# rust-bio/rust-bio

Measured on AMD Instinct MI355X. Metric: GCUPS (SW) + FM-index queries/sec, higher is better.
Workload: dtype int16; 1 GPU; 1000000 x 150 bp synthetic read pairs per GPU, Aligner::local affine-gap (-5,-1,+1,-1), score+coords+traceback ops (BASELINE configs[1]); pairs_per_gpu=1000000, read_len=150, parallelism=shard1

## Files before the change

### rust-bio_amd/csrc/sw_fill_pk16.inc

```
#include <type_traits>

#include "sw_kernels.h"

namespace bgsw {
namespace pk16 {

typedef uint32_t pk;

typedef short s16x2 __attribute__((ext_vector_type(2)));
typedef unsigned short u16x2 __attribute__((ext_vector_type(2)));
typedef _Float16 h16x2 __attribute__((ext_vector_type(2)));
__device__ __forceinline__ s16x2 as_s(pk v) { return __builtin_bit_cast(s16x2, v); }
__device__ __forceinline__ u16x2 as_u(pk v) { return __builtin_bit_cast(u16x2, v); }
__device__ __forceinline__ pk bits(s16x2 v) { return __builtin_bit_cast(pk, v); }
__device__ __forceinline__ pk bits(u16x2 v) { return __builtin_bit_cast(pk, v); }
__device__ __forceinline__ pk pk_adds(pk a, pk b) { return bits(__builtin_elementwise_add_sat(as_s(a), as_s(b))); }
__device__ __forceinline__ pk pk_max(pk a, pk b) { return bits(__builtin_elementwise_max(as_s(a), as_s(b))); }
__device__ __forceinline__ pk pk_max3h(pk a, pk b, pk c) {
    const h16x2 x = __builtin_bit_cast(h16x2, a), y = __builtin_bit_cast(h16x2, b), z = __builtin_bit_cast(h16x2, c);
    return __builtin_bit_cast(pk, __builtin_elementwise_maximum(__builtin_elementwise_maximum(x, y), z));
}
__device__ __forceinline__ pk pk_min(pk a, pk b) { return bits(__builtin_elementwise_min(as_s(a), as_s(b))); }
__device__ __forceinline__ pk pk_add_u16(pk a, pk b) { return bits((u16x2)(as_u(a) + as_u(b))); }
__device__ __forceinline__ pk pk_sub_u16(pk a, pk b) { return bits((u16x2)(as_u(a) - as_u(b))); }
__device__ __forceinline__ pk pk_subs_u16(pk a, pk b) { return bits(__builtin_elementwise_sub_sat(as_u(a), as_u(b))); }
__device__ __forceinline__ pk pk_mad_u16(pk a, pk b, pk c) { return bits((u16x2)(as_u(a) * as_u(b) + as_u(c))); }
__device__ __forceinline__ pk dup16(int32_t v) { return ((uint32_t)v & 0xffffu) | ((uint32_t)v << 16); }
__device__ __forceinline__ pk bfi(pk mask, pk a, pk b) { return (a & mask) | (b & ~mask); }
__device__ __forceinline__ pk nz_mask(pk v, pk one) { return pk_sub_u16(pk_subs_u16(one, v), one); }

template <int LP>
__device__ __forceinline__ void scan_first_max(int ll, int64_t& v, uint32_t& idx) {
#pragma unroll
    for (int off = 1; off < LP; off <<= 1) {
        const int64_t ov = __shfl_up(v, off, LP);
        const uint32_t oi = (uint32_t)__shfl_up((int)idx, off, LP);
        if (ll >= off && !(v > ov)) {
            v = ov;
            idx = oi;
        }
    }
}

constexpr int32_t kFloor16 = -2048;

enum { CZ = 0, CF = 1, CI = 2 };
template <int R, int LP, int MODE, int XP, int XS, int YP, int YS, bool LF = false, int FR = 0>
__device__ __forceinline__ void sw_fill_pk16_body(const SwArgs& a) {
    constexpr bool FAST = MODE == 0;
    constexpr int PW = 64 / LP;
    constexpr int NW = tb_words(R);
    constexpr int NH = (R + 2) / 3;
    constexpr bool NARROW = true, LOCAL = XP == CZ && XS == CZ && YP == CZ && YS == CZ;
    constexpr bool ROW0_ZERO = YP == CZ && YS == CZ;
    constexpr int SH = 4;
    constexpr int32_t NEGS = kFloor16 * 16;
    constexpr pk CLEAN = 0xfff0fff0u, FLOORK = 0x80008000u, ONE = 0x00010001u;
    static_assert(LP == 16 || LP == 32, "lanes per pair");
    static_assert(R >= 1 && R <= 12, "rows per lane");
    static_assert(!LF || LOCAL, "LF is a flavour of the local kernel");
    static_assert(FR >= 0 && FR <= 2 && (!FR || LF), "the frame is a cell of the LF flavour");
    (void)NARROW;
    (void)LOCAL;
    constexpr int kTileStride = 20;
    constexpr int kParkDw = 64 * (4 * R + NH + 1), kTileDw = 2 * 64 * kTileStride;
    constexpr int kWaveDw = kParkDw > kTileDw ? kParkDw : kTileDw;
    __shared__ __align__(16) pk s_lds[4 * kWaveDw];
    pk* const wave_lds = s_lds + (threadIdx.x >> 6) * kWaveDw;

    const int lane = threadIdx.x & 63;
    const uint32_t wv = blockIdx.x * (blockDim.x >> 6) + (threadIdx.x >> 6);
    if ((uint64_t)wv * 2 * PW >= a.n_pairs) return;
    if (MODE == 2 && a.len_stats && a.len_stats[0] == a.len_stats[2] && a.len_stats[1] == a.len_stats[3]) return;
    const int g = lane / LP, ll = lane % LP;
    const SwScoring sc = a.sc;
    const SwGeom geo = a.g;
    auto scl = [](int32_t v) -> int32_t { return max(v, kFloor16) * 16; };
    const int32_t go_s = sc.go * 16, xs_s = sc.xs <= kFloor16 ? -(1 << 30) : sc.xs * 16;
    (void)xs_s;
    constexpr int32_t K_XS = C_XS << 1, K_MATCH = C_MATCH << 1, K_SUBST = C_SUBST << 1, K_INS = C_INS << 1,
                      K_DEL = C_DEL << 1, K_XP = C_XP << 1;
    constexpr pk NOFLAG = 0xfffefffeu;
    const pk GE = dup16(sc.ge * 16);
    const pk GOT_I = dup16(sc.go * 16 + K_INS + 1), GOT_D = dup16(sc.go * 16 + K_DEL + 1);
    const pk MISK = dup16((sc.mismatch * 16) | K_SUBST);
    const pk DELTA = dup16(((sc.match * 16) | K_MATCH) - ((sc.mismatch * 16) | K_SUBST));
    const pk XS16 = dup16(scl(sc.xs)), YS16 = dup16(scl(sc.ys));
    const pk XSCAP = sc.xs <= kFloor16 ? FLOORK : 0x7fff7fffu, YSCAP = sc.ys <= kFloor16 ? FLOORK : 0x7fff7fffu;
    (void)XS16; (void)YS16; (void)XSCAP; (void)YSCAP;
    const pk MISC = dup16(-((sc.mismatch * 16) | K_SUBST));
    (void)MISC;
    auto fr = [](int32_t c) -> pk { return (uint32_t)c * 0x10001u; };
    const int32_t gF = -16 * sc.ge, BF = pk16_frame_bias(sc);
    const pk GF = fr(gF);
    const pk KGOI = fr(sc.go * 16 + K_INS + 1 + gF), KGOD = fr(sc.go * 16 + K_DEL + 1 + gF);
    const pk KSUB = fr(((sc.mismatch * 16) | K_SUBST) + 2 * gF);
    const pk KREB = fr(gF * (R - 1));
    (void)GF; (void)KGOI; (void)KGOD; (void)KSUB; (void)KREB;
    pk C16 = dup16(16), C32 = dup16(32), C1024 = dup16(1024);
    asm volatile("" : "+s"(C16), "+s"(C32), "+s"(C1024));

    const uint32_t pA = (2 * wv) * PW + g, pB = (2 * wv + 1) * PW + g;
    const bool okA = pA < a.n_pairs, okB = pB < a.n_pairs;
    uint32_t mA = 0, nA = 0, mB = 0, nB = 0;
    uint64_t xoA = 0, yoA = 0, xoB = 0, yoB = 0;
    const uint32_t* perm = a.slot_perm();
    if (okA) {
        const uint64_t r = a.pair0 + (perm ? perm[pA] : pA);
        xoA = a.x_off[r];
        yoA = a.y_off[r];
        mA = (uint32_t)(a.x_off[r + 1] - xoA);
        nA = (uint32_t)(a.y_off[r + 1] - yoA);
        if (len_over(geo, mA, nA)) mA = nA = 0;
    }
    if (okB) {
        const uint64_t r = a.pair0 + (perm ? perm[pB] : pB);
        xoB = a.x_off[r];
        yoB = a.y_off[r];
        mB = (uint32_t)(a.x_off[r + 1] - xoB);
        nB = (uint32_t)(a.y_off[r + 1] - yoB);
        if (len_over(geo, mB, nB)) mB = nB = 0;
    }
    const bool same = okA && okB && mA == mB && nA == nB;
    const bool two = okA && okB && !same;
    const bool m_last0 = LF || __all(!okA || mA % R == 0);
    if (MODE == 0 && !m_last0) return;
    if (MODE == 1 && m_last0) return;
    if (MODE == 2 && !__any(two)) return;
    const uint64_t job_words = tb_job_words(geo.nstrips, geo.nsteps, NW);

    auto do_pass = [&](const int pass) {
        const bool pair_ok = pass == 0 ? okA : two;
        const uint32_t P0 = pass == 0 ? pA : pB, P1 = (pass == 0 && !same) ? pA : pB;
        const uint32_t m = !pair_ok ? 0 : (pass == 0 ? mA : mB), n = !pair_ok ? 0 : (pass == 0 ? nA : nB);
        const uint64_t xs0 = pass == 0 ? xoA : xoB, ys0 = pass == 0 ? yoA : yoB;
        const uint64_t xs1 = (pass == 0 && !same) ? xoA : xoB, ys1 = (pass == 0 && !same) ? yoA : yoB;
        const uint8_t* x0 = a.x + xs0;
        const uint8_t* x1 = a.x + xs1;
        const bool packed = a.packed != 0;
        auto y_pair = [&](uint32_t col) -> pk {
            if (packed) return sym2(a.y, ys0 + col) | (sym2(a.y, ys1 + col) << 16);
            return (uint32_t)a.y[ys0 + col] | ((uint32_t)a.y[ys1 + col] << 16);
        };
        const uint32_t Q0 = pair_ok ? P0 : 0, Q1 = pair_ok ? P1 : 0;
        uint32_t* tb0 = (uint32_t*)a.tb + (size_t)(Q0 / PW) * job_words + ((Q0 % PW) * LP + ll) * 16u;
        uint32_t* tb1 = (uint32_t*)a.tb + (size_t)(Q1 / PW) * job_words + ((Q1 % PW) * LP + ll) * 16u;
        int32_t* aux0 = a.aux + (size_t)Q0 * geo.aux_stride;
        int32_t* aux1 = a.aux + (size_t)Q1 * geo.aux_stride;
        int32_t* gLx0 = aux0 + geo.off_Lx();
        int32_t* gLx1 = aux1 + geo.off_Lx();

        uint32_t m_w = m, n_w = n;
#pragma unroll
        for (int o = 32; o; o >>= 1) {
            m_w = max(m_w, (uint32_t)__shfl_xor((int)m_w, o));
            n_w = max(n_w, (uint32_t)__shfl_xor((int)n_w, o));
        }
        (void)m_w;
        n_w = (uint32_t)__builtin_amdgcn_readfirstlane((int)n_w);
        const uint32_t nsteps_w = n_w ? n_w + LP - 1 : 0;

        int32_t fold0;
        uint32_t lx0;
        col0_fold(sc, m, fold0, lx0);
        int32_t Sn0 = sc.ys;
        uint32_t Ly0 = n;
        int32_t S0n = 0;
        uint32_t sb0n = (ROW0_ZERO && n) ? row0_cell(sc, n).sbits : (uint32_t)TB_START;
        if (pair_ok && ll == 0) {
            const int32_t v = m ? (int32_t)col0_cell(sc, m, m, fold0).sbits : (int32_t)TB_START;
            aux0[0] = v;
            aux1[0] = v;
            if (m == 0) {
                if (LP == 16) {
                    *(uint8_t*)gLx0 = (uint8_t)lx0;
                    *(uint8_t*)gLx1 = (uint8_t)lx0;
                } else {
                    *(uint16_t*)gLx0 = (uint16_t)lx0;
                    *(uint16_t*)gLx1 = (uint16_t)lx0;
                }
            }
        }

        const uint32_t rb = (uint32_t)ll * R;
        const int32_t mrow = (int32_t)m - (int32_t)rb - 1;
        pk Sl[R], Dl[R], Il[R], SnR[R], SnB[R], Ly[R], px[R];
        uint64_t nib0S = 0, nib0I = 0;
        uint64_t xw0 = 0, xw1 = 0;
        if (packed && pair_ok && rb < m) {
            const uint32_t* p0 = (const uint32_t*)a.x + ((xs0 + rb) >> 4);
            const uint32_t* p1 = (const uint32_t*)a.x + ((xs1 + rb) >> 4);
            xw0 = (((uint64_t)p0[1] << 32) | p0[0]) >> (2 * ((uint32_t)(xs0 + rb) & 15u));
            xw1 = (((uint64_t)p1[1] << 32) | p1[0]) >> (2 * ((uint32_t)(xs1 + rb) & 15u));
        }
#pragma unroll
        for (int r = 0; r < R; r++) {
            const uint32_t i = rb + r + 1;
            px[r] = 0;
            Sl[r] = Dl[r] = Il[r] = SnR[r] = SnB[r] = FLOORK;
            Ly[r] = 0;
            if (pair_ok && i <= m) {
                px[r] = packed ? (((uint32_t)(xw0 >> (2 * r)) & 3u) | (((uint32_t)(xw1 >> (2 * r)) & 3u) << 16))
                               : ((uint32_t)x0[i - 1] | ((uint32_t)x1[i - 1] << 16));
                const Col0 c = col0_cell(sc, i, m, fold0);
                Sl[r] = dup16(scl(c.S));
                Il[r] = dup16(scl(c.I) | K_INS);
                nib0S |= (uint64_t)c.sbits << (4 * r);
                nib0I |= (uint64_t)c.ibits << (4 * r);
                if (YS != CI && c.S + sc.ys > NEG) {
                    SnR[r] = dup16(scl(c.S + sc.ys));
                    Ly[r] = dup16((int32_t)n);
                }
            }
        }
        pk diag0 = dup16((pair_ok && rb < m) ? scl(col0_S(sc, rb, m, fold0)) : NEGS);
        if (FR) {
            const int32_t off0 = BF + gF * ((int32_t)ll - 1);
#pragma unroll
            for (int r = 0; r < R; r++) {
                const pk o = fr(off0 + gF * r);
                Sl[r] = (pair_ok && rb + r + 1 <= m) ? Sl[r] + o : o;
                Il[r] += o;
                Dl[r] = 0;
            }
            diag0 = fr(off0 - gF) + ((pair_ok && rb < m) ? dup16(scl(col0_S(sc, rb, m, fold0))) : 0u);
        }

        pk S_out = FLOORK, I_out = FLOORK, cm_out = FLOORK, ca_out = 0, q_out = 0;
        pk ychunk = 0, ychunk_nx = 0;
        pk hwlast[NH];
#pragma unroll
        for (int k = 0; k < NH; k++) hwlast[k] = 0;
        pk lx_n = dup16((int32_t)lx0);
        pk* tileA = wave_lds + (0 * 64 + lane) * kTileStride;
        pk* tileB = wave_lds + (1 * 64 + lane) * kTileStride;
        uint32_t lxaccA = lx0 << (LP == 16 ? 24 : 16), lxaccB = lxaccA;
        if (pair_ok && (uint32_t)ll < n) ychunk_nx = y_pair((uint32_t)ll);

        auto merge_rows = [&](uint32_t blockbase) {
            const pk lybase = dup16((int32_t)(n - blockbase - 16u + (uint32_t)ll));
#pragma unroll
            for (int r = 0; r < R; r++) {
                const pk nr = pk_max(SnR[r], SnB[r] & CLEAN);
                const pk msk = nz_mask(nr ^ SnR[r], ONE);
                Ly[r] = bfi(msk, pk_add_u16(lybase, SnB[r] & 0x000f000fu), Ly[r]);
                SnR[r] = nr;
                SnB[r] = FLOORK;
            }
        };

        constexpr uint32_t tsteps = tb_tile_steps(NW);
        auto store_tile = [&](uint32_t s_any) {
            if (!pair_ok) return;
            const uint32_t off = (s_any / tsteps) * 1024u;
#pragma unroll
            for (int k = 0; k < 4; k++) {
                *(uint4*)&tb0[off + 4 * k] = *(const uint4*)&tileA[4 * k];
                *(uint4*)&tb1[off + 4 * k] = *(const uint4*)&tileB[4 * k];
            }
        };
        uint32_t s_all = pair_ok ? n + (uint32_t)ll : 0u;
#pragma unroll
        for (int o = 32; o; o >>= 1) s_all = min(s_all, (uint32_t)__shfl_xor((int)s_all, o));
        s_all = (uint32_t)__builtin_amdgcn_readfirstlane((int)s_all);
        auto run_steps = [&](auto mr_tag) {
        constexpr int MRk = decltype(mr_tag)::value;
        auto step = [&](auto allon_tag, auto fast_tag, const uint32_t s) {
            constexpr bool ALLON = decltype(allon_tag)::value;
            constexpr bool FB = decltype(fast_tag)::value;
            constexpr bool FOLD = XS != CI && !FB;
            if ((s & (LP - 1)) == 0) {
                ychunk = ychunk_nx;
                const uint32_t nb = s + LP + ll;
                if (pair_ok && nb < n) ychunk_nx = y_pair(nb);
            }
            pk S_up = (pk)wave_shr1((int)S_out, (int)S_out), I_up = (pk)wave_shr1((int)I_out, (int)I_out);
            if (FR) {
                S_up -= KREB;
                I_up -= KREB;
            }
            pk cm = FLOORK, ca = 0;
            if (FOLD) {
                cm = (pk)wave_shr1((int)cm_out, (int)cm_out);
                ca = (pk)wave_shr1((int)ca_out, (int)ca_out);
            }
            pk q = (pk)wave_shr1((int)q_out, (int)q_out);
            const uint32_t j = s + 1 - (uint32_t)ll;
            const bool col_ok = ALLON || (pair_ok && (j - 1) < n);
            const pk F0 = fr(BF + gF * (int32_t)s);
            (void)F0;
            if (ll == 0) {
                q = ychunk;
                S_up = FR ? F0 - GF : 0u;
                I_up = FR ? 0u : FLOORK;
                cm = FLOORK;
                ca = 0;
                if (!ROW0_ZERO && col_ok) {
                    const Row0 c = row0_cell(sc, j);
                    int32_t S0 = c.S;
                    uint32_t sb = c.sbits;
                    if (j == n && Sn0 > S0) {
                        S0 = Sn0;
                        sb = TB_YCLIP_SUFFIX;
                    } else if (S0 + sc.ys > Sn0) {
                        Sn0 = S0 + sc.ys;
                        Ly0 = n - j;
                    }
                    S0n = S0;
                    sb0n = sb;
                    S_up = dup16(scl(S0));
                }
            }
            ychunk = (pk)wave_shl1((int)ychunk, (int)ychunk);

            if (col_ok) {
                const pk sprio = dup16((int32_t)(15u - (s & 15u)));
                pk diag = diag0;
                diag0 = S_up;
                pk hw[NH];
                const pk ca_in = ca;
                pk cmk = cm | 0x000f000fu;
                pk snap = cmk;
                pk XKEY = dup16(K_XP);
                if (XP == CF || (XP == CZ && YP != CZ))
                    XKEY = dup16(scl(sc.xp + max(sc.yp, sc.go + sc.ge * ((int32_t)j - 1))) | K_XP);
#pragma unroll
                    for (int r = 0; r < R; r++) {
                        const bool maybe_m = MRk < 0 || r == MRk;
                        const bool is_m = MRk < 0 ? (r == mrow) : (r == MRk && mrow == MRk);
                        const pk e = pk_subs_u16(ONE, px[r] ^ q);
                        const pk Fr = F0 + (uint32_t)r * GF;
                        (void)Fr;
                        const pk m_key = FR == 2 ? pk_mad_u16(e, DELTA, diag) + KSUB
                                         : FR    ? pk_max(pk_mad_u16(e, DELTA, diag) + KSUB, Fr)
                                         : LF    ? pk_subs_u16(pk_mad_u16(e, DELTA, diag), MISC)
                                                 : pk_adds(diag, pk_mad_u16(e, DELTA, MISK));
                        const pk Iv_t = FR ? pk_max(I_up, S_up + KGOI) : pk_max(pk_adds(I_up, GE), pk_adds(S_up, GOT_I));
                        const pk Dv_t = FR ? pk_max(Dl[r], Sl[r] + KGOD) : pk_max(pk_adds(Dl[r], GE), pk_adds(Sl[r], GOT_D));
                        const pk Iv = Iv_t & NOFLAG, Dv = Dv_t & NOFLAG;
                        pk kb = FR == 2 ? pk_max3h(m_key, Fr, Dv_t) : pk_max(m_key, Dv_t);
                        if (XP != CI && !LF) kb = pk_max(kb, XKEY);
                        kb = FR == 2 ? pk_max3h(kb, Iv_t, Iv_t) : pk_max(kb, Iv_t);
                        if (FOLD && maybe_m)
                            kb = pk_max(kb, is_m ? ((cmk & CLEAN) | (0x00010001u * K_XS)) : FLOORK);
                        const pk best = kb & CLEAN;
                        diag = Sl[r];
                        Sl[r] = best;
                        Dl[r] = Dv;
                        Il[r] = Iv;
                        S_up = best;
                        I_up = Iv;
                        if (FOLD) {
                            if (maybe_m) snap = is_m ? cmk : snap;
                            const pk fv = XS == CZ ? best : pk_min(pk_adds(best, XS16), XSCAP);
                            cmk = pk_max(cmk, fv | (0x00010001u * (uint32_t)(14 - r)));
                        }
                        if (YS != CI) {
                            const pk t1 = YS == CZ ? best : pk_min(pk_adds(best, YS16), YSCAP);
                            SnB[r] = pk_max(SnB[r], FR ? best - (Fr - sprio) : t1 | sprio);
                        }
                        const pk c5 = pk_mad_u16(Dv_t & ONE, C16, (kb & 0x000e000eu) | (Iv_t & ONE));
                        if (r % 3 == 0)
                            hw[r / 3] = c5;
                        else
                            hw[r / 3] = pk_mad_u16(c5, r % 3 == 1 ? C32 : C1024, hw[r / 3]);
                    }
                if (FOLD) {
                    const pk mbase = dup16(mrow - 14);
                    const pk lo = cmk & 0x000f000fu, slo = snap & 0x000f000fu;
                    if (mrow >= 0 && mrow < R) {
                        const pk is15 = nz_mask(slo ^ 0x000f000fu, ONE);
                        lx_n = bfi(is15, pk_add_u16(slo, mbase), ca_in);
                        if (LP == 16) {
                            lxaccA = __builtin_amdgcn_perm(lx_n, lxaccA, 0x04030201u);
                            lxaccB = __builtin_amdgcn_perm(lx_n, lxaccB, 0x06030201u);
                            if ((j & 3u) == 3u || j == n) {
                                const uint32_t sh = 8u * (3u - (j & 3u));
                                ((uint32_t*)gLx0)[j >> 2] = lxaccA >> sh;
                                ((uint32_t*)gLx1)[j >> 2] = lxaccB >> sh;
                            }
                        } else {
                            lxaccA = __builtin_amdgcn_perm(lx_n, lxaccA, 0x05040302u);
                            lxaccB = __builtin_amdgcn_perm(lx_n, lxaccB, 0x07060302u);
                            if ((j & 1u) == 1u || j == n) {
                                const uint32_t sh = 16u * (1u - (j & 1u));
                                ((uint32_t*)gLx0)[j >> 1] = lxaccA >> sh;
                                ((uint32_t*)gLx1)[j >> 1] = lxaccB >> sh;
                            }
                        }
                    }
                    {
                        const pk is15 = nz_mask(lo ^ 0x000f000fu, ONE);
                        ca = bfi(is15, pk_add_u16(lo, mbase), ca_in);
                    }
                    cm = cmk & CLEAN;
                }
                constexpr pk INV = 0x00010001u * (17u | (17u << 5) | (17u << 10));
                constexpr pk INV_LAST = 0x00010001u * ((R % 3 == 0) ? (17u | (17u << 5) | (17u << 10))
                                                      : (R % 3 == 1) ? 17u : (17u | (17u << 5)));
#pragma unroll
                for (int k = 0; k < NH; k++) {
                    hw[k] ^= (k == NH - 1) ? INV_LAST : INV;
                    hwlast[k] = hw[k];
                }
                const pk h0 = hw[0], h1 = NH > 1 ? hw[NH > 1 ? 1 : 0] : 0u;
                const uint32_t slot = (s % tsteps) * NW;
                if (NW == 1) {
                    tileA[slot] = __builtin_amdgcn_perm(h1, h0, 0x05040100u);
                    tileB[slot] = __builtin_amdgcn_perm(h1, h0, 0x07060302u);
                } else {
                    const pk h2 = hw[NH > 2 ? 2 : 0], h3 = NH > 3 ? hw[NH > 3 ? 3 : 0] : 0u;
                    *(uint2*)&tileA[slot] = make_uint2(__builtin_amdgcn_perm(h1, h0, 0x05040100u),
                                                       __builtin_amdgcn_perm(h3, h2, 0x05040100u));
                    *(uint2*)&tileB[slot] = make_uint2(__builtin_amdgcn_perm(h1, h0, 0x07060302u),
                                                       __builtin_amdgcn_perm(h3, h2, 0x07060302u));
                }
                S_out = S_up;
                I_out = I_up;
                if (FOLD) {
                    cm_out = cm;
                    ca_out = ca;
                }
                q_out = q;
            }
            if (s % tsteps == tsteps - 1) store_tile(s);
            if (YS != CI && (s & 15u) == 15u) merge_rows(s & ~15u);
        };
        uint32_t s = 0;
        const uint32_t s_on = min((uint32_t)(LP - 1), nsteps_w), s_off = max(s_on, min(s_all, nsteps_w));
        constexpr std::false_type no{};
        constexpr std::true_type yes{};
        constexpr std::bool_constant<LF> fast{};
        for (; s < s_on; s++) step(no, fast, s);
        for (; s + 1 < s_off; s += 2) {
            step(yes, fast, s);
            step(yes, fast, s + 1);
        }
        for (; s < s_off; s++) step(yes, fast, s);
        for (; s < nsteps_w; s++) step(no, fast, s);
        };
        run_steps(std::integral_constant<int, (FAST && !LF) ? R - 1 : -1>{});
        if (nsteps_w % tsteps) store_tile(nsteps_w - 1);
        if (YS != CI && nsteps_w) merge_rows((nsteps_w - 1) & ~15u);

        pk* park = wave_lds + lane;
        const pk offl = FR ? fr(BF + gF * ((int32_t)ll + (int32_t)n - 1)) : 0u;
#pragma unroll
        for (int r = 0; r < R; r++) {
            park[(0 * R + r) * 64] = FR ? Sl[r] - (offl + (uint32_t)r * GF) : Sl[r];
            park[(1 * R + r) * 64] = FR ? Il[r] - (offl + (uint32_t)r * GF) : Il[r];
            park[(2 * R + r) * 64] = SnR[r];
            park[(3 * R + r) * 64] = Ly[r];
        }
#pragma unroll
        for (int k = 0; k < NH; k++) park[(4 * R + k) * 64] = hwlast[k];
        park[(4 * R + NH) * 64] = lx_n;
        const int nhalf = (pair_ok && P1 != P0) ? 2 : 1;
        const int nhalf_w = __any(nhalf == 2) ? 2 : 1;
#pragma unroll 1
        for (int h = 0; h < nhalf_w; h++) {
            if (h >= nhalf) continue;
            const uint32_t hs = 16u * (uint32_t)h;
            int32_t* aux = h ? aux1 : aux0;
            int32_t* gLy = aux + geo.off_Ly();
            uint8_t* gBits = (uint8_t*)(aux + geo.off_bits());
            const uint32_t strip = 0;
            struct HalfS {
                const pk* p;
                uint32_t hs;
                __device__ int32_t operator[](int r) const { return (int32_t)(int16_t)(p[r * 64] >> hs); }
            };
            struct HalfU {
                const pk* p;
                uint32_t hs;
                __device__ uint32_t operator[](int r) const { return (p[r * 64] >> hs) & 0xffffu; }
            };
            int32_t Sl_u[R];
#pragma unroll
            for (int r = 0; r < R; r++) Sl_u[r] = (int32_t)(int16_t)(park[r * 64] >> hs);
            const HalfS Il_u{park + 1 * R * 64, hs}, Sn_u{park + 2 * R * 64, hs};
            const HalfU Ly_u{park + 3 * R * 64, hs};
            const uint32_t lx_n_u = (park[(4 * R + NH) * 64] >> hs) & 0xffffu;
            int64_t e_carry = INT64_MIN;
            uint32_t sbf_carry = TB_START, sb2_carry = TB_START;
            int64_t c1v = INT64_MIN, c2v = INT64_MIN;
            uint32_t c1i = 0, c2i = 0;
            auto cell_of = [&](int r) -> uint32_t {
                const uint32_t c = (park[(4 * R + r / 3) * 64] >> (hs + 5 * (r % 3))) & 31u;
                const uint32_t mv = (c >> 1) & 7u;
                return ((LF && mv == 0) ? (uint32_t)C_XP : mv) | ((c & 1u) << 3) | (c & 16u);
            };
            {
                constexpr bool EPI_FOLD_PRE = LF;
                int32_t(&Sl)[R] = Sl_u;
                const HalfS& Il = Il_u;
                const HalfS& Sn = Sn_u;
                const HalfU& Ly = Ly_u;
                const uint32_t lx_n = lx_n_u;
#include "sw_epilogue.inc"
            }
        }
    };
    do_pass(MODE == 2 ? 1 : 0);
}

template <int R, int LP, int XP, int XS, int YP, int YS, bool LF, int FR = 0>
__global__ __launch_bounds__(256) __attribute__((amdgpu_waves_per_eu(R <= 10 ? 3 : 2, R <= 10 ? 3 : 2))) void sw_fill_pk16_kernel(const SwArgs a) {
    sw_fill_pk16_body<R, LP, 0, XP, XS, YP, YS, LF, FR>(a);
}
template <int R, int LP, int XP, int XS, int YP, int YS, bool LF, int FR = 0>
__global__ __launch_bounds__(256) __attribute__((amdgpu_waves_per_eu(R <= 10 ? 3 : 2, R <= 10 ? 3 : 2))) void sw_fill_pk16_rest_kernel(const SwArgs a) {
    sw_fill_pk16_body<R, LP, 1, XP, XS, YP, YS, LF, FR>(a);
}
template <int R, int LP, int XP, int XS, int YP, int YS, bool LF, int FR = 0>
__global__ __launch_bounds__(256) __attribute__((amdgpu_waves_per_eu(R <= 10 ? 3 : 2, R <= 10 ? 3 : 2))) void sw_fill_pk16_second_kernel(const SwArgs a) {
    sw_fill_pk16_body<R, LP, 2, XP, XS, YP, YS, LF, FR>(a);
}

}
}

#define BG_PK16_CASE(LP_, R_)                                                                          \
    if (lp == LP_ && r == R_)                                                                         \
        return which == 0   ? pk16::sw_fill_pk16_kernel<R_, LP_, XP_, XS_, YP_, YS_, LF_, FR_>        \
               : which == 1 ? pk16::sw_fill_pk16_rest_kernel<R_, LP_, XP_, XS_, YP_, YS_, LF_, FR_>   \
                            : pk16::sw_fill_pk16_second_kernel<R_, LP_, XP_, XS_, YP_, YS_, LF_, FR_>;
```

### rust-bio_amd/csrc/sw_kernels.h

```cpp
#ifndef BG_SW_KERNELS_H
#define BG_SW_KERNELS_H
#include <type_traits>

#include "bg_common.h"

namespace bgsw {

constexpr int32_t NEG = BG_MIN_SCORE;

enum : uint32_t {
    TB_START = 0, TB_INS = 1, TB_DEL = 2, TB_SUBST = 3, TB_MATCH = 4,
    TB_XCLIP_PREFIX = 5, TB_XCLIP_SUFFIX = 6, TB_YCLIP_PREFIX = 7, TB_YCLIP_SUFFIX = 8
};
enum : uint32_t { C_XS = 7, C_MATCH = 6, C_SUBST = 5, C_INS = 3, C_DEL = 2, C_XP = 1, C_YP = 0 };
constexpr int32_t kNarrowFloor = -(1 << 26);
constexpr int32_t kNarrowKeyFloor = (int32_t)0x80000000;

enum { SCORE_PARAMS = 0, SCORE_LDS = 1, SCORE_GLOBAL = 2 };
constexpr int kMaxLdsAlphabet = 64;

struct SwScoring {
    int32_t go, ge, xp, xs, yp, ys;
    int32_t match, mismatch;
};

__host__ __device__ inline int32_t pk16_frame_bias(const SwScoring& sc) {
    const int32_t g = -16 * sc.ge;
    int32_t b = 2 * g;
    const int32_t lows[3] = {-((sc.mismatch * 16) | (int32_t)(C_SUBST << 1)), -(sc.go * 16 + (int32_t)(C_INS << 1)),
                             -(sc.go * 16 + (int32_t)(C_DEL << 1))};
    for (int32_t v : lows) b = b > v ? b : v;
    return (b + 15) & ~15;
}
inline bool pk16_frame_fits(const SwScoring& sc, uint32_t max_ylen, int r, int lp) {
    if (sc.ge > 0 || sc.match < 0) return false;
    const int64_t g = -16ll * sc.ge, nsteps = (int64_t)max_ylen + lp - 1;
    return 16ll * sc.match * max_ylen + pk16_frame_bias(sc) + g * (r + nsteps) + 15 < 0x8000;
}
inline bool pk16_max3_fits(const SwScoring& sc, uint32_t max_ylen, int r, int lp) {
    if (sc.ge > 0 || sc.match < 0) return false;
    const int64_t g = -16ll * sc.ge, nsteps = (int64_t)max_ylen + lp - 1;
    return 16ll * sc.match * max_ylen + pk16_frame_bias(sc) + g * (r + nsteps) + 15 < 0x7c00;
}

enum : uint32_t {
    TBF_K1 = 0,
    TBF_K1P = 1,
    TBF_K1P_LF = 2,
    TBF_K1_LF = 3
};

struct SwGeom {
    uint32_t lp, r, nsteps, nstrips, m_cap, n_cap, aux_stride;
    uint32_t tb_fmt;
    uint32_t r_inv;
    uint32_t lp_shift;
    __host__ __device__ uint32_t off_Ly() const { return 4; }
    __host__ __device__ uint32_t off_Lx() const { return 4 + (m_cap + 1); }
    __host__ __device__ uint32_t off_bits() const { return 4 + (m_cap + 1) + (n_cap + 1); }
    __host__ __device__ static uint32_t stride_for(uint32_t m_cap, uint32_t n_cap) {
        return 4 + (m_cap + 1) + (n_cap + 1) + (m_cap + 1 + 3) / 4;
    }
};

__device__ __forceinline__ bool len_over(const SwGeom& g, uint32_t m, uint32_t n) { return m > g.m_cap || n > g.n_cap; }

__host__ __device__ constexpr int tb_words(int r) { return (r + 5) / 6; }
__host__ __device__ constexpr uint32_t tb_tile_steps(int nw) { return 16u / (uint32_t)nw; }
__host__ __device__ inline uint64_t tb_job_words(uint32_t nstrips, uint32_t nsteps, int nw) {
    const uint64_t g = (uint64_t)nstrips * nsteps, t = tb_tile_steps(nw);
    return (g + t - 1) / t * 1024ull;
}
__host__ __device__ inline uint64_t tb_word_off(uint64_t g, uint32_t lane, int nw) {
    const uint32_t t = tb_tile_steps(nw);
    return (g / t) * 1024ull + lane * 16u + (uint32_t)(g % t) * (uint32_t)nw;
}

struct SwArgs {
    const uint8_t* x;
    const uint64_t* x_off;
    const uint8_t* y;
    const uint64_t* y_off;
    uint64_t pair0;
    uint32_t n_pairs;
    SwScoring sc;
    const int32_t* table;
    const uint8_t* code_map;
    int32_t alpha;
    void* tb;
    int32_t* aux;
    int4* bnd;
    const uint32_t* perm;
    const uint32_t* len_stats;
    const uint32_t* n_eff;
    __device__ const uint32_t* slot_perm() const {
        if (!perm) return nullptr;
        if (len_stats && len_stats[0] == len_stats[2] && len_stats[1] == len_stats[3]) return nullptr;
        return perm;
    }
    SwGeom g;
    bg_alignment_t* out;
    uint8_t* ops;
    uint64_t ops_stride;
    int32_t mode;
    int32_t filter_clips;
    int32_t packed;
};
__device__ __forceinline__ uint32_t sym2(const uint8_t* stream, uint64_t s) {
    return (((const uint32_t*)stream)[s >> 4] >> (2 * ((uint32_t)s & 15u))) & 3u;
}

struct Col0 {
    int32_t S, I;
    uint32_t sbits, ibits;
};
__device__ __forceinline__ Col0 col0_cell(const SwScoring& sc, uint32_t i, uint32_t m, int32_t fold) {
    Col0 c;
    if (i == 1) {
        c.I = sc.go;
        c.ibits = TB_START;
    } else {
        const int32_t i_score = sc.go + sc.ge * ((int32_t)i - 1);
        const int32_t c_score = sc.xp + sc.go;
        if (i_score > c_score) {
            c.I = i_score;
            c.ibits = TB_INS;
        } else {
            c.I = c_score;
            c.ibits = TB_XCLIP_PREFIX;
        }
    }
    if (i == m) {
        c.S = fold;
        c.sbits = TB_XCLIP_SUFFIX;
    } else {
        c.S = NEG;
        c.sbits = TB_START;
    }
    if (c.I > c.S) {
        c.S = c.I;
        c.sbits = TB_INS;
    }
    if (sc.xp > c.S) {
        c.S = sc.xp;
        c.sbits = TB_XCLIP_PREFIX;
    }
    return c;
}
__device__ __forceinline__ void col0_fold(const SwScoring& sc, uint32_t m, int32_t& fold, uint32_t& lx0) {
    fold = NEG;
    lx0 = 0;
    if (m >= 2) {
        const Col0 c = col0_cell(sc, 1, m, NEG);
        if (c.S + sc.xs > fold) {
            fold = c.S + sc.xs;
            lx0 = m - 1;
        }
    }
}
__device__ __forceinline__ int32_t col0_S(const SwScoring& sc, uint32_t i, uint32_t m, int32_t fold0) {
    if (i == 0) return 0;
    return col0_cell(sc, i, m, fold0).S;
}

struct Row0 {
    int32_t S, D;
    uint32_t sbits, dbits;
};
__device__ __forceinline__ Row0 row0_cell(const SwScoring& sc, uint32_t j) {
    Row0 c;
    if (j == 1) {
        c.D = sc.go;
        c.dbits = TB_START;
    } else {
        const int32_t d_score = sc.go + sc.ge * ((int32_t)j - 1);
        const int32_t c_score = sc.yp + sc.go;
        if (d_score > c_score) {
            c.D = d_score;
            c.dbits = TB_DEL;
        } else {
            c.D = c_score;
            c.dbits = TB_YCLIP_PREFIX;
        }
    }
    if (c.D > sc.yp) {
        c.S = c.D;
        c.sbits = TB_DEL;
    } else {
        c.S = sc.yp;
        c.sbits = TB_YCLIP_PREFIX;
    }
    return c;
}

__device__ __forceinline__ uint32_t s_nibble_of_code(uint32_t code) {
    switch (code) {
        case C_MATCH: return TB_MATCH;
        case C_SUBST: return TB_SUBST;
        case C_INS: return TB_INS;
        case C_DEL: return TB_DEL;
        case C_XP: return TB_XCLIP_PREFIX;
        case C_YP: return TB_YCLIP_PREFIX;
        default: return TB_XCLIP_SUFFIX;
    }
}

typedef void (*sw_fill_fn)(const SwArgs);

#define BG_K1_SHAPES(X) X(16, 2) X(16, 4) X(16, 6) X(16, 8) X(16, 10) X(16, 12) X(32, 8) X(32, 10) X(32, 12) X(64, 8)
#define BG_K1_TABLE_SHAPES(X) X(16, 6) X(16, 12) X(32, 12) X(64, 8)
#define BG_K1_TABLE_LDS_NARROW_SHAPES(X) BG_K1_TABLE_SHAPES(X) X(16, 8) X(16, 10)
#define BG_K1P_SHAPES(X) X(16, 2) X(16, 4) X(16, 5) X(16, 6) X(16, 8) X(16, 10) X(16, 12) X(32, 8) X(32, 10) X(32, 12)
#define BG_K1P_LOCAL_SHAPES(X)                                                                                    \
    X(16, 2) X(16, 3) X(16, 4) X(16, 5) X(16, 6) X(16, 7) X(16, 8) X(16, 9) X(16, 10) X(16, 11) X(16, 12) \
    X(32, 7) X(32, 8) X(32, 9) X(32, 10) X(32, 11) X(32, 12)

#define BG_SW_FILLS(X) \
    X(K1) X(K1_LOCAL) X(K1_LF) X(K1_LDS) X(K1_LDS_LOCAL) X(K1_GLOBAL) X(K1P_CUSTOM) X(K1P_GLOBAL) X(K1P_SEMIGLOBAL) X(K1P_LOCAL) X(K1P_LF) X(K1P_LF_FRAMED) X(K1P_LF_FRAMED_MAX3)
enum SwFill {
#define BG_X(F) FILL_##F,
    BG_SW_FILLS(BG_X)
#undef BG_X
};
#define BG_X(F) sw_fill_fn sw_fill_get_##F(bool narrow, int lp, int r, int which);
BG_SW_FILLS(BG_X)
#undef BG_X

}
#endif
```

Baseline: 2251 GCUPS.

## Trim per-cell ops in FR==2 pk16 cell: symbol shift, D floor, paired row-max

For the framed max3 packed-int16 Smith-Waterman cell, symbols are pre-shifted by 8 bits so the match/mismatch delta comes from one saturating subtract against DELTA, replacing a multiply-add. The frame floor moves into the D computation so the later max3 chain needs fewer operations, and the per-row suffix maximum (SnB) is updated once every two steps with a three-way max over both steps' scores. This cuts VALU work in the inner cell, with a new guard restricting the delta to 0..256 and an alignment step so the step pairs start on even indices. Compile-time KO bits allow each idea to be switched off.

```diff
diff --git a/rust-bio_amd/csrc/sw_fill_pk16.inc b/rust-bio_amd/csrc/sw_fill_pk16.inc
--- a/rust-bio_amd/csrc/sw_fill_pk16.inc
+++ b/rust-bio_amd/csrc/sw_fill_pk16.inc
@@ -1,6 +1,10 @@
 #include <type_traits>
 
 #include "sw_kernels.h"
+
+#ifndef PK16_CELL_KO
+#define PK16_CELL_KO 0
+#endif
 
 namespace bgsw {
 namespace pk16 {
@@ -97,6 +101,10 @@
     const pk KSUB = fr(((sc.mismatch * 16) | K_SUBST) + 2 * gF);
     const pk KREB = fr(gF * (R - 1));
     (void)GF; (void)KGOI; (void)KGOD; (void)KSUB; (void)KREB;
+    constexpr bool DFLOOR = FR == 2 && !(PK16_CELL_KO & 1);
+    constexpr bool SYMHI = FR == 2 && !(PK16_CELL_KO & 2);
+    constexpr bool ROWMAX2 = FR == 2 && !(PK16_CELL_KO & 4);
+    constexpr int SYM_SH = SYMHI ? 8 : 0;
     pk C16 = dup16(16), C32 = dup16(32), C1024 = dup16(1024);
     asm volatile("" : "+s"(C16), "+s"(C32), "+s"(C1024));
 
@@ -139,8 +147,8 @@
         const uint8_t* x1 = a.x + xs1;
         const bool packed = a.packed != 0;
         auto y_pair = [&](uint32_t col) -> pk {
-            if (packed) return sym2(a.y, ys0 + col) | (sym2(a.y, ys1 + col) << 16);
-            return (uint32_t)a.y[ys0 + col] | ((uint32_t)a.y[ys1 + col] << 16);
+            if (packed) return (sym2(a.y, ys0 + col) | (sym2(a.y, ys1 + col) << 16)) << SYM_SH;
+            return ((uint32_t)a.y[ys0 + col] | ((uint32_t)a.y[ys1 + col] << 16)) << SYM_SH;
         };
         const uint32_t Q0 = pair_ok ? P0 : 0, Q1 = pair_ok ? P1 : 0;
         uint32_t* tb0 = (uint32_t*)a.tb + (size_t)(Q0 / PW) * job_words + ((Q0 % PW) * LP + ll) * 16u;
@@ -202,6 +210,7 @@
             if (pair_ok && i <= m) {
                 px[r] = packed ? (((uint32_t)(xw0 >> (2 * r)) & 3u) | (((uint32_t)(xw1 >> (2 * r)) & 3u) << 16))
                                : ((uint32_t)x0[i - 1] | ((uint32_t)x1[i - 1] << 16));
+                px[r] <<= SYM_SH;
                 const Col0 c = col0_cell(sc, i, m, fold0);
                 Sl[r] = dup16(scl(c.S));
                 Il[r] = dup16(scl(c.I) | K_INS);
@@ -265,8 +274,10 @@
         s_all = (uint32_t)__builtin_amdgcn_readfirstlane((int)s_all);
         auto run_steps = [&](auto mr_tag) {
         constexpr int MRk = decltype(mr_tag)::value;
-        auto step = [&](auto allon_tag, auto fast_tag, const uint32_t s) {
+        auto step = [&](auto allon_tag, auto fast_tag, auto trip_tag, const uint32_t s) {
             constexpr bool ALLON = decltype(allon_tag)::value;
+            constexpr int TRIP = decltype(trip_tag)::value;
+            static_assert(!TRIP || (ALLON && ROWMAX2), "trips are pairs of unpredicated steps of the FR == 2 cell");
             constexpr bool FB = decltype(fast_tag)::value;
             constexpr bool FOLD = XS != CI && !FB;
             if ((s & (LP - 1)) == 0) {
@@ -328,22 +339,28 @@
                     for (int r = 0; r < R; r++) {
                         const bool maybe_m = MRk < 0 || r == MRk;
                         const bool is_m = MRk < 0 ? (r == mrow) : (r == MRk && mrow == MRk);
-                        const pk e = pk_subs_u16(ONE, px[r] ^ q);
+                        const pk e = pk_subs_u16(SYMHI ? DELTA : ONE, px[r] ^ q);
                         const pk Fr = F0 + (uint32_t)r * GF;
                         (void)Fr;
-                        const pk m_key = FR == 2 ? pk_mad_u16(e, DELTA, diag) + KSUB
+                        pk dk = diag + KSUB;
+                        if (SYMHI && !(PK16_CELL_KO & 8)) asm("" : "+v"(dk));
+                        const pk m_key = SYMHI   ? e + dk
+                                         : FR == 2 ? pk_mad_u16(e, DELTA, diag) + KSUB
                                          : FR    ? pk_max(pk_mad_u16(e, DELTA, diag) + KSUB, Fr)
                                          : LF    ? pk_subs_u16(pk_mad_u16(e, DELTA, diag), MISC)
                                                  : pk_adds(diag, pk_mad_u16(e, DELTA, MISK));
                         const pk Iv_t = FR ? pk_max(I_up, S_up + KGOI) : pk_max(pk_adds(I_up, GE), pk_adds(S_up, GOT_I));
-                        const pk Dv_t = FR ? pk_max(Dl[r], Sl[r] + KGOD) : pk_max(pk_adds(Dl[r], GE), pk_adds(Sl[r], GOT_D));
+                        const pk Dv_t = DFLOOR ? pk_max3h(Dl[r], Sl[r] + KGOD, Fr)
+                                        : FR   ? pk_max(Dl[r], Sl[r] + KGOD)
+                                               : pk_max(pk_adds(Dl[r], GE), pk_adds(Sl[r], GOT_D));
                         const pk Iv = Iv_t & NOFLAG, Dv = Dv_t & NOFLAG;
-                        pk kb = FR == 2 ? pk_max3h(m_key, Fr, Dv_t) : pk_max(m_key, Dv_t);
+                        pk kb = DFLOOR ? m_key : FR == 2 ? pk_max3h(m_key, Fr, Dv_t) : pk_max(m_key, Dv_t);
                         if (XP != CI && !LF) kb = pk_max(kb, XKEY);
-                        kb = FR == 2 ? pk_max3h(kb, Iv_t, Iv_t) : pk_max(kb, Iv_t);
+                        kb = DFLOOR ? pk_max3h(kb, Dv_t, Iv_t) : FR == 2 ? pk_max3h(kb, Iv_t, Iv_t) : pk_max(kb, Iv_t);
                         if (FOLD && maybe_m)
                             kb = pk_max(kb, is_m ? ((cmk & CLEAN) | (0x00010001u * K_XS)) : FLOORK);
                         const pk best = kb & CLEAN;
+                        const pk best_prev = Sl[r];
                         diag = Sl[r];
                         Sl[r] = best;
                         Dl[r] = Dv;
@@ -357,7 +374,10 @@
                         }
                         if (YS != CI) {
                             const pk t1 = YS == CZ ? best : pk_min(pk_adds(best, YS16), YSCAP);
-                            SnB[r] = pk_max(SnB[r], FR ? best - (Fr - sprio) : t1 | sprio);
+                            if (TRIP == 2)
+                                SnB[r] = pk_max3h(SnB[r], best_prev - (Fr - GF - sprio - ONE), best - (Fr - sprio));
+                            else if (TRIP == 0)
+                                SnB[r] = pk_max(SnB[r], FR ? best - (Fr - sprio) : t1 | sprio);
                         }
                         const pk c5 = pk_mad_u16(Dv_t & ONE, C16, (kb & 0x000e000eu) | (Iv_t & ONE));
                         if (r % 3 == 0)
@@ -431,13 +451,17 @@
         constexpr std::false_type no{};
         constexpr std::true_type yes{};
         constexpr std::bool_constant<LF> fast{};
-        for (; s < s_on; s++) step(no, fast, s);
+        constexpr std::integral_constant<int, 0> single{};
+        constexpr std::integral_constant<int, ROWMAX2 ? 1 : 0> first{};
+        constexpr std::integral_constant<int, ROWMAX2 ? 2 : 0> second{};
+        for (; s < s_on; s++) step(no, fast, single, s);
+        if (ROWMAX2 && (s & 1u) && s < s_off) step(yes, fast, single, s++);
         for (; s + 1 < s_off; s += 2) {
-            step(yes, fast, s);
-            step(yes, fast, s + 1);
-        }
-        for (; s < s_off; s++) step(yes, fast, s);
-        for (; s < nsteps_w; s++) step(no, fast, s);
+            step(yes, fast, first, s);
+            step(yes, fast, second, s + 1);
+        }
+        for (; s < s_off; s++) step(yes, fast, single, s);
+        for (; s < nsteps_w; s++) step(no, fast, single, s);
         };
         run_steps(std::integral_constant<int, (FAST && !LF) ? R - 1 : -1>{});
         if (nsteps_w % tsteps) store_tile(nsteps_w - 1);
diff --git a/rust-bio_amd/csrc/sw_kernels.h b/rust-bio_amd/csrc/sw_kernels.h
--- a/rust-bio_amd/csrc/sw_kernels.h
+++ b/rust-bio_amd/csrc/sw_kernels.h
@@ -37,8 +37,12 @@
     const int64_t g = -16ll * sc.ge, nsteps = (int64_t)max_ylen + lp - 1;
     return 16ll * sc.match * max_ylen + pk16_frame_bias(sc) + g * (r + nsteps) + 15 < 0x8000;
 }
+__host__ __device__ inline int32_t pk16_delta(const SwScoring& sc) {
+    return ((sc.match * 16) | (int32_t)(C_MATCH << 1)) - ((sc.mismatch * 16) | (int32_t)(C_SUBST << 1));
+}
 inline bool pk16_max3_fits(const SwScoring& sc, uint32_t max_ylen, int r, int lp) {
     if (sc.ge > 0 || sc.match < 0) return false;
+    if (pk16_delta(sc) < 0 || pk16_delta(sc) > 256) return false;
     const int64_t g = -16ll * sc.ge, nsteps = (int64_t)max_ylen + lp - 1;
     return 16ll * sc.match * max_ylen + pk16_frame_bias(sc) + g * (r + nsteps) + 15 < 0x7c00;
 }
```

Result: faster. 2347 GCUPS (median of 6 runs) (+4.3%).
